# lanl/jaybenne

Measured on AMD Instinct MI355X. Metric: particle-histories/s (whole node) on stepdiff, higher is better.
Workload: dtype f64

## Files before the change

jaybenne_amd/csrc/jb_kernel_imc.hpp:

```cpp
#pragma once

#include "jb_kernels.hpp"

namespace jb {

#ifndef JB_IMC_WAVES_PER_SIMD_UNIFORM
#define JB_IMC_WAVES_PER_SIMD_UNIFORM 4
#endif
#ifndef JB_IMC_WAVES_PER_SIMD
#define JB_IMC_WAVES_PER_SIMD 4
#endif
#ifndef JB_IMC_WAVES_PER_SIMD_LOWD
#define JB_IMC_WAVES_PER_SIMD_LOWD 4
#endif
#ifndef JB_IMC_NT_STORES
#define JB_IMC_NT_STORES 0
#endif
#ifndef JB_IMC_MASKED_NUDGE
#define JB_IMC_MASKED_NUDGE 1
#endif
#ifndef JB_IMC_SERVICE_BUDGET
#define JB_IMC_SERVICE_BUDGET 96
#endif

struct ImcArgs {
  const DevMesh *Mp;
  DevParams P;
  DevSwarm S;
  double t_start, dt;
  long long first, last;
  unsigned long long *counters;
  const int *nbr_dq;
};

enum { IS_IDLE = 0, IS_RUN = 1, IS_DONE = 2, IS_DONE_RAW = 3 };
#ifndef JB_IMC_WIDE_LOG
#define JB_IMC_WIDE_LOG 1
#endif
constexpr bool kWideLog = JB_IMC_WIDE_LOG != 0;


template <int NDIM, bool TALLY, bool NOABS, bool UNIFORM>
__global__ void __launch_bounds__(kBlock, NDIM < 3 ? JB_IMC_WAVES_PER_SIMD_LOWD
                                          : UNIFORM ? JB_IMC_WAVES_PER_SIMD_UNIFORM : JB_IMC_WAVES_PER_SIMD)
    k_imc_cell(const DevMesh *__restrict__, DevParams, DevSwarm, double, double, long long, long long,
               unsigned long long *, const int *) {
  const ImcArgs &A = *(const ImcArgs *)__builtin_amdgcn_kernarg_segment_ptr();
  const DevMesh &M = *A.Mp;
  const DevParams &P = A.P;
  const DevSwarm &S = A.S;
  const double t_start = A.t_start, dt = A.dt;
  const long long first = A.first, last = A.last;
  unsigned long long *const counters = g1(A.counters);
  (void)A.nbr_dq;
  constexpr bool multi_d = NDIM >= 2, three_d = NDIM == 3;
  __shared__ double lds_tally[TALLY ? kLdsTally : 1];
  const bool tally_in_lds = TALLY && (long long)M.nblocks * M.ntot <= (long long)kLdsTally;
  if constexpr (TALLY) {
    if (tally_in_lds)
      for (int q = threadIdx.x; q < M.nblocks * (int)M.ntot; q += blockDim.x) lds_tally[q] = 0.0;
  }
  constexpr bool kWide = kWideLog && NOABS;
  constexpr bool kMasked = JB_IMC_MASKED_NUDGE != 0;
  load_math_tables<false, !kWide, false, true, kWide>();

  constexpr int kServiceBudget = JB_IMC_SERVICE_BUDGET;
  const double vv = P.c;
  const double t_end = t_start + dt;
  const int lane = threadIdx.x & 63;
  unsigned long long *queue = counters + CNT_QUEUE;
  const long long per_q = (last - first + kQueues - 1) / kQueues;
  int cur = blockIdx.x % kQueues;
  int tried = 0;
  bool more = true;

  unsigned int c_census = 0, c_abs = 0, c_esc = 0, c_out = 0;
  unsigned long long c_evp = 0;
  unsigned int c_service = 0;

  const int sy = (int)sgpr_copy(8u * (unsigned)M.ni), sz = (int)sgpr_copy(8u * (unsigned)(M.ni * M.nj));
  const unsigned blk_bytes = 16u * (unsigned)M.ntot;
  const char *const lam_abs0 = (const char *)sgpr_copy_ptr(M.lam_base);
  const char *const lam_sc0 = (const char *)sgpr_copy_ptr(M.lam_base + M.ntot);
  const double inv_ni = 1.0 / (double)M.ni, inv_ninj = 1.0 / (double)(M.ni * M.nj);
  const double inv_blk_bytes = 1.0 / (double)blk_bytes;

  int ls = IS_IDLE;
  long long n = 0;
  LcgRng rng(0);
  int b = 0, status = ST_ACTIVE;
  unsigned qoff = 0u;
  double px = 0, py = 0, pz = 0;
  double ox = 0, oy = 0, oz = 0;
  double drem = 0;
  CellGeom cg{0, 0, 0, 0, 0, 0, 0};
  if constexpr (UNIFORM) {
    const double d0 = uniform_f64(M.blk_dx[0]), d1 = uniform_f64(M.blk_dx[1]), d2 = uniform_f64(M.blk_dx[2]);
    cg.hx = 0.5 * d0; cg.hy = 0.5 * d1; cg.hz = 0.5 * d2;
    cg.mx = cg.hx - kEpsImc * d0; cg.my = cg.hy - kEpsImc * d1; cg.mz = cg.hz - kEpsImc * d2;
    cg.dxp = dmin(d0, dmin(d1, d2));
  }
  double lam_a = 0.0, lam_s = 0.0;
  JB_INV_STMT(bool inv_collided = false;)

  auto fetch_lam = [&]() {
    if constexpr (!NOABS) lam_a = *(gcptr)(lam_abs0 + qoff);
    lam_s = *(gcptr)(lam_sc0 + qoff);
  };
  auto bind_block = [&](int blk) {
    if constexpr (UNIFORM) return;
    const double d0 = ((gcptr)M.blk_dx)[3 * blk], d1 = ((gcptr)M.blk_dx)[3 * blk + 1],
                 d2 = ((gcptr)M.blk_dx)[3 * blk + 2];
    cg.hx = 0.5 * d0; cg.hy = 0.5 * d1; cg.hz = 0.5 * d2;
    cg.mx = cg.hx - kEpsImc * d0; cg.my = cg.hy - kEpsImc * d1; cg.mz = cg.hz - kEpsImc * d2;
    cg.dxp = dmin(d0, dmin(d1, d2));
  };
  auto block_of = [&]() { return (int)(((double)qoff + 4.0) * inv_blk_bytes); };
  auto cell_of = [&](int &i, int &j, int &k) {
    const int q = (int)((qoff - (unsigned)b * blk_bytes) >> 3);
    k = three_d ? (int)(((double)q + 0.5) * inv_ninj) : 0;
    const int r = q - k * (M.ni * M.nj);
    j = multi_d ? (int)(((double)r + 0.5) * inv_ni) : 0;
    i = r - j * M.ni;
  };
  auto centre = [&](int blk, int d, int idx) {
    const double dxd = ((gcptr)M.blk_dx)[3 * blk + d];
    const int first_d = d == 0 ? M.is : (d == 1 ? M.js : M.ks);
    const double x0 = ((gcptr)M.blk_xmin)[3 * blk + d] - (double)first_d * dxd;
    return fma((double)idx + 0.5, dxd, x0);
  };
  auto materialise = [&](double &x, double &y, double &z, int &i, int &j, int &k) {
    cell_of(i, j, k);
    x = centre(b, 0, i) + px;
    y = multi_d ? centre(b, 1, j) + py : py;
    z = three_d ? centre(b, 2, k) + pz : pz;
  };
  auto localise = [&](double x, double y, double z, int i, int j, int k) {
    px = x - centre(b, 0, i);
    py = multi_d ? y - centre(b, 1, j) : y;
    pz = three_d ? z - centre(b, 2, k) : z;
    qoff = (unsigned)b * blk_bytes + ((unsigned)cidx(M, k, j, i) << 3);
  };
  bool abs_pos = false;
  auto relocate = [&]() {
    double x, y, z;
    int i, j, k;
    materialise(x, y, z, i, j, k);
    if (!apply_swarm_bcs<NDIM>(M, x, y, z, ox, oy, oz)) {
      status = ST_ESCAPED;
      px = x; py = y; pz = z;
      abs_pos = true;
      ls = IS_DONE;
      return;
    }
    const int g = find_block<NDIM>(M, x, y, z);
    const int li = M.local_index[g];
    if (li < 0) {
      status = ST_OUTGOING;
      b = g;
      px = x; py = y; pz = z;
      abs_pos = true;
      ls = IS_DONE;
      return;
    }
    b = li;
    bind_block(b);
    Blk B;
    load_block(M, b, B);
    xtoijk<NDIM>(M, B, x, y, z, i, j, k);
    localise(x, y, z, i, j, k);
    ls = (drem > 0.0) ? IS_RUN : IS_DONE;
    fetch_lam();
  };

  for (;;) {
    ++c_service;
    if (ls == IS_DONE || ls == IS_DONE_RAW) {
      double x = px, y = py, z = pz;
      int ip = 0, jp = 0, kp = 0;
      if (!abs_pos) {
        b = block_of();
        materialise(x, y, z, ip, jp, kp);
      }
      double t = drem, vx = ox, vy = oy, vz = oz;
      if (ls == IS_DONE) {
        t = fma(-drem, P.rc, t_end);
        vx *= vv; vy *= vv; vz *= vv;
      }
      int bw = b;
      if (!abs_pos && (status == ST_ACTIVE || status == ST_OUTGOING_ABSORBED) && !M.owned[b]) {
        if (status == ST_ACTIVE) status = ST_OUTGOING;
        bw = M.gid[b];
      }
#if JB_IMC_NT_STORES
#define JB_WST(p, v) __builtin_nontemporal_store((v), (p))
#else
#define JB_WST(p, v) (*(p) = (v))
#endif
      JB_WST(&g1(S.blk)[n], bw);
      JB_WST(&g1(S.t)[n], t);
      JB_WST(&g1(S.x)[n], x); JB_WST(&g1(S.y)[n], y); JB_WST(&g1(S.z)[n], z);
      JB_WST(&g1(S.vx)[n], vx); JB_WST(&g1(S.vy)[n], vy); JB_WST(&g1(S.vz)[n], vz);
      JB_WST(&g1(S.ip)[n], ip); JB_WST(&g1(S.jp)[n], jp); JB_WST(&g1(S.kp)[n], kp);
      JB_WST(&g1(S.status)[n], status);
      JB_WST(&g1(S.rng)[n], (uint64_t)rng.s);
#undef JB_WST
      if (status == ST_ACTIVE) {
        ++c_census;
        if constexpr (TALLY) {
          const double dv = (8.0 * cg.hx) * cg.hy * cg.hz;
          const int q = (int)((qoff - (unsigned)b * blk_bytes) >> 3);
          if (tally_in_lds) atomicAdd(&lds_tally[b * (int)M.ntot + q], g1(S.w)[n] / dv);
          else atomicAdd(&M.tally[b][q], g1(S.w)[n] / dv);
        }
      } else if (status == ST_ABSORBED) {
        ++c_abs;
      } else if (status == ST_ESCAPED) {
        ++c_esc;
      } else {
        ++c_out;
      }
      ls = IS_IDLE;
      abs_pos = false;
    }
    {
      const unsigned long long idle = __ballot(ls == IS_IDLE);
      if (idle != 0ull && more) {
        const int leader = __ffsll((long long)idle) - 1;
        const int want = __popcll(idle);
        unsigned long long base = 0;
        if (lane == leader) base = atomicAdd(&queue[cur * kQueueStride], (unsigned long long)want);
        base = __shfl(base, leader, 64);
        const long long q_first = first + (long long)cur * per_q;
        long long q_last = q_first + per_q;
        if (q_last > last) q_last = last;
        const long long cand = q_first + (long long)base + __popcll(idle & ((1ull << lane) - 1ull));
        if (q_first + (long long)base + want >= q_last) {
          cur = (cur + 1) % kQueues;
          if (++tried == kQueues) more = false;
        }
        if (ls == IS_IDLE && cand < q_last && g1(S.status)[cand] == ST_ACTIVE) {
          n = cand;
          rng.s = g1(S.rng)[n];
          b = g1(S.blk)[n];
          bind_block(b);
          const double t = g1(S.t)[n];
          const double x = g1(S.x)[n], y = g1(S.y)[n], z = g1(S.z)[n];
          ox = g1(S.vx)[n]; oy = g1(S.vy)[n]; oz = g1(S.vz)[n];
          status = ST_ACTIVE;
          Blk B;
          load_block(M, b, B);
          int i, j, k;
          xtoijk<NDIM>(M, B, x, y, z, i, j, k);
          localise(x, y, z, i, j, k);
          if (t < t_end) {
            drem = vv * (t_end - t);
            ox *= P.rc; oy *= P.rc; oz *= P.rc;
            ls = IS_RUN;
          } else {
            drem = t;
            ls = IS_DONE_RAW;
          }
          fetch_lam();
        }
      }
    }
    const int running = __popcll(__ballot(ls == IS_RUN));
    if (running == 0) {
      if (__ballot(ls != IS_IDLE) != 0ull || more) continue;
      break;
    }
    int waste = 0;

    int thresh = 1;
    int nrun = running;
    while (nrun >= thresh) {
      const bool run = ls == IS_RUN;
      const bool cross = run && lam_s < 0.0;
      const bool stepping = run && !cross;
      const unsigned long long cross_m =
          __builtin_amdgcn_ballot_w64(ls == IS_RUN) & __builtin_amdgcn_ballot_w64(lam_s < 0.0);
      c_evp += (1ull << 40) + (unsigned long long)(nrun - __popcll(cross_m));
      if (cross_m != 0ull) {
        if (cross) {
          JB_INV_OFF_BLOCK(JB_INV_FAM_IMC_CELL, inv_collided, false, block_of(), 0, 0, 0, px, py, pz, n, S.id, (void)0);
          const int code = __double2hiint(lam_s);
          if ((code & kGhostTable) == 0) {
            b = block_of();
            relocate();
          } else {
            const int fx = (code << 15) & (int)0x80000000u, fy = (code << 14) & (int)0x80000000u,
                      fz = (code << 13) & (int)0x80000000u;
            px = __hiloint2double(__double2hiint(px) ^ fx, __double2loint(px));
            ox = __hiloint2double(__double2hiint(ox) ^ fx, __double2loint(ox));
            if (multi_d) {
              py = __hiloint2double(__double2hiint(py) ^ fy, __double2loint(py));
              oy = __hiloint2double(__double2hiint(oy) ^ fy, __double2loint(oy));
            }
            if (three_d) {
              pz = __hiloint2double(__double2hiint(pz) ^ fz, __double2loint(pz));
              oz = __hiloint2double(__double2hiint(oz) ^ fz, __double2loint(oz));
            }
            qoff = (unsigned)__double2loint(lam_s);
            if constexpr (!UNIFORM) {
              if (code & (kGhostCoarser | kGhostFiner))
                qoff = cross_level<NDIM>(code, qoff, sy, sz, cg, px, py, pz);
            }
            fetch_lam();
            if (!(drem > 0.0)) ls = IS_DONE;
          }
        }
      }
      JB_INV_STMT(bool inv_bad = false;)
      JB_INV_STMT({
        int ib = -1, ii = 0, ij = 0, ik = 0, ax = 0;
        const double pp[3] = {px, py, pz}, hh[3] = {cg.hx, cg.hy, cg.hz};
        const bool pos = inv::local_position_ok(NDIM, pp, hh, ax);
        const unsigned cell = (qoff % blk_bytes) >> 3;
        const bool idx = cell < (unsigned)M.ntot &&
                         inv::cell_interior(M, (unsigned long long)(qoff / blk_bytes) * (unsigned long long)M.ntot + cell,
                                            ib, ii, ij, ik);
        JB_INV_PASS_PRED(JB_INV_FAM_IMC_CELL, stepping, pos, idx, ax, ib, ii, ij, ik, px, py, pz, n, S.id,
                         { inv_bad = true; ls = IS_IDLE; });
      })
      if (stepping JB_INV_STMT(&& !inv_bad)) {
        bool is_absorbed, is_scattered, hit_any;
        unsigned long long hit_m;
        imc_step_cell<NDIM, NOABS, UNIFORM, kWide, kMasked>(cg, sy, sz, lam_a, lam_s, rng, drem, px, py, pz, ox, oy, oz,
                                                     qoff, is_absorbed, is_scattered, hit_any, &hit_m, fetch_lam);
        const bool alive = drem > 0.0, census = !alive;
        bool collide = is_absorbed || is_scattered;
        bool off = false;
        const unsigned long long at_face_m =
            hit_m & (__builtin_amdgcn_ballot_w64(collide) | ~__builtin_amdgcn_ballot_w64(alive));
        const bool at_face = __builtin_amdgcn_inverse_ballot_w64(at_face_m);
        if (at_face_m != 0ull) {
          asm volatile("; collision or census next to a cell face" ::: "memory");
          if (at_face) off = lam_s < 0.0;
        }
        collide = collide && !off;
        JB_INV_STMT(inv_collided = collide;)
        if (!NOABS && is_absorbed && collide) {
          b = block_of();
          if (M.owned[b]) {
            atomicAdd(&M.edelta[b][(qoff - (unsigned)b * blk_bytes) >> 3], g1(S.w)[n]);
            status = ST_ABSORBED;
          } else {
            status = ST_OUTGOING_ABSORBED;
          }
          ls = IS_DONE;
        } else {
          if (is_scattered && collide) scatter_dir<true>(rng, ox, oy, oz);
          if (census && !off) ls = IS_DONE;
        }
      }
      nrun = __popcll(__ballot(ls == IS_RUN));
      waste += running - nrun;
      if (waste >= kServiceBudget) thresh = 65;
    }
  }

  if constexpr (TALLY) {
    if (tally_in_lds) {
      __syncthreads();
      for (int q = threadIdx.x; q < M.nblocks * (int)M.ntot; q += blockDim.x) {
        const double v = lds_tally[q];
        if (v != 0.0) atomicAdd(&M.tally[q / (int)M.ntot][q % (int)M.ntot], v);
      }
    }
  }
  unsigned long long r_census = wave_sum(c_census), r_abs = wave_sum(c_abs), r_esc = wave_sum(c_esc),
                     r_out = wave_sum(c_out);
  if (lane == 0) {
    if (r_census) atomicAdd(&counters[CNT_CENSUS], r_census);
    if (r_abs) atomicAdd(&counters[CNT_ABSORBED], r_abs);
    if (r_esc) atomicAdd(&counters[CNT_ESCAPED], r_esc);
    if (r_out) atomicAdd(&counters[CNT_OUTGOING], r_out);
    atomicAdd(&counters[CNT_EVENTS], c_evp & ((1ull << 40) - 1ull));
    atomicAdd(&counters[CNT_PASSES], c_evp >> 40);
    atomicAdd(&counters[CNT_SERVICE], (unsigned long long)c_service);
  }
}

}
```

jaybenne_amd/csrc/jb_physics.hpp:

```cpp
#pragma once

#include <float.h>
#include <hip/hip_runtime.h>

#include "jb_math.hpp"
#include "jb_rng.hpp"

namespace jb {

constexpr double kEps = 10.0 * DBL_EPSILON;
constexpr double kEpsImc = 1.0e6 * kEps;
constexpr double kEpsDdmc = 1.0e8 * kEps;
constexpr double kLamExt = 0.7104;
constexpr double kTwoPi = 2.0 * 3.14159265358979323846;

__device__ __forceinline__ double dmin(double a, double b) { return (b < a) ? b : a; }

__device__ __forceinline__ bool fuzzy_equal(double a, double b, double c, double eps) {
  return fabs(a - b) < c * eps;
}

__device__ __forceinline__ void face_iso_dir(double vv, double xi1, double xi2, double &v1,
                                             double &v2, double &v3) {
  const double mu = m_sqrt(xi1);
  const double om = 1.0 - mu * mu;
  const double nu = (om > 0.0) ? m_sqrt(om > 0.0 ? om : 1.0) : 0.0;
  double sn, cs;
  m_sincos2pi(xi2, sn, cs);
  v1 = vv * mu;
  v2 = vv * nu * cs;
  v3 = vv * nu * sn;
}

template <class Rng>
__device__ __forceinline__ void sample_face_iso_dir(double vv, Rng &rng, double &v1, double &v2,
                                                    double &v3) {
  const double xi1 = rng.drand();
  const double xi2 = rng.drand();
  face_iso_dir(vv, xi1, xi2, v1, v2, v3);
}

template <class Rng>
__device__ __forceinline__ void scatter(Rng &rng, double vv, double &vx, double &vy, double &vz) {
  double xi1, xi2;
  rng.drand2(xi1, xi2);
  const double mu = fma(2.0, xi1, -1.0);
  const double st = m_sqrt(1.0 - mu * mu);
  double sn, cs;
  m_sincos2pi(xi2, sn, cs);
  vx = vv * st * cs;
  vy = vv * st * sn;
  vz = vv * mu;
}

template <class Rng>
__device__ __forceinline__ double sample_planck_energy(Rng &rng, double sb, double temp) {
  constexpr double kPi = 3.14159265358979323846;
  const double xi0 = rng.drand();
  const double rhs = xi0 * ((kPi * kPi) * (kPi * kPi)) / 90.0;
  double ll = 1.0;
  for (int l = 1; l < 100; ++l) {
    double lhs = 0.0;
    for (int j = 1; j <= l; ++j) {
      const double dj = (double)j;
      lhs += 1.0 / ((dj * dj) * (dj * dj));
    }
    if (lhs >= rhs) {
      ll = (double)l;
      break;
    }
  }
  const double xi1 = rng.drand();
  const double xi2 = rng.drand();
  const double xi3 = rng.drand();
  const double xi4 = rng.drand();
  return -(1.0 / ll) * m_log(xi1 * xi2 * xi3 * xi4) * sb * temp;
}

struct Step {
  double t_start, dt;
  double ff, aa, ss, vv, dx_push;
  double rvv;
  double ffaa, sig;
  double xl, yl, zl, xu, yu, zu;
  double Px_l, Py_l, Pz_l, Px_u, Py_u, Pz_u;
  double t, x, y, z, vx, vy, vz;
  int ip, jp, kp;
  bool is_absorbed, is_scattered, is_rejected;
  int pend;
  double pz1, pz2;
};

__device__ __forceinline__ void imc_cell_mfp(double ff, double aa, double ss, double &lam_abs,
                                             double &lam_sc) {
  const double rmin = DBL_MIN;
  lam_abs = 1.0 / (ff * aa + rmin);
  lam_sc = 1.0 / (ss + (1.0 - ff) * aa + rmin);
}

template <int NDIM, bool NOABS = false, class Rng>
__device__ __forceinline__ void imc_step_core(Step &s, double lam_abs, double lam_sc, Rng &rng) {
  constexpr bool multi_d = NDIM >= 2, three_d = NDIM == 3;
  double dx_abs = 0.0;
  if constexpr (NOABS) rng.skip();
  else dx_abs = -lam_abs * m_log(rng.drand());
  const double dx_sc = -lam_sc * m_log(rng.drand());
  const double dx_end = s.vv * ((s.t_start + s.dt) - s.t);
  double dx_push = dmin(s.dx_push, dx_end);
  {
    const double d = m_div(s.vv * ((s.vx > 0.0 ? s.xu : s.xl) - s.x), s.vx);
    dx_push = (s.vx != 0.0) ? dmin(dx_push, d) : dx_push;
  }
  if (multi_d) {
    const double d = m_div(s.vv * ((s.vy > 0.0 ? s.yu : s.yl) - s.y), s.vy);
    dx_push = (s.vy != 0.0) ? dmin(dx_push, d) : dx_push;
  }
  if (three_d) {
    const double d = m_div(s.vv * ((s.vz > 0.0 ? s.zu : s.zl) - s.z), s.vz);
    dx_push = (s.vz != 0.0) ? dmin(dx_push, d) : dx_push;
  }

  s.is_absorbed = NOABS ? false : (dx_abs < dx_push) && (dx_abs < dx_sc);
  s.is_scattered = !s.is_absorbed && (dx_sc < dx_push);

  const double dt_push = m_div_r(s.is_absorbed ? dx_abs : (s.is_scattered ? dx_sc : dx_push), s.vv,
                                 s.rvv);

  s.t += dt_push;
  s.x += s.vx * dt_push;
  s.y += (multi_d ? 1.0 : 0.0) * s.vy * dt_push;
  s.z += (three_d ? 1.0 : 0.0) * s.vz * dt_push;

  const double fdx = kEpsImc * (s.xu - s.xl);
  const double fdy = kEpsImc * (s.yu - s.yl);
  const double fdz = kEpsImc * (s.zu - s.zl);
  if (fabs(s.x - s.xl) < fdx) s.x = s.xl - fdx;
  if (fabs(s.x - s.xu) < fdx) s.x = s.xu + fdx;
  if (multi_d && fabs(s.y - s.yl) < fdy) s.y = s.yl - fdy;
  if (multi_d && fabs(s.y - s.yu) < fdy) s.y = s.yu + fdy;
  if (three_d && fabs(s.z - s.zl) < fdz) s.z = s.zl - fdz;
  if (three_d && fabs(s.z - s.zu) < fdz) s.z = s.zu + fdz;
}

__device__ __forceinline__ void idx_step(int &i, bool hi, bool lo) {
  i += (int)hi;
  i -= (int)lo;
}

struct ImcCell {
  double xl, xu, yl, yu, zl, zu;
  double fdx, fdy, fdz;
};
template <int NDIM, bool NOABS, bool LEAN = false, class Rng>
__device__ __forceinline__ void imc_step_fast(const ImcCell &c, double vv, double rvv, double t_end,
                                              double dx_push0, double lam_abs, double lam_sc,
                                              Rng &rng, double &t, double &x, double &y, double &z,
                                              double vx, double vy, double vz, int &ip, int &jp,
                                              int &kp, bool &is_absorbed, bool &is_scattered) {
  constexpr bool multi_d = NDIM >= 2, three_d = NDIM == 3;
  double dx_abs = 0.0;
  if constexpr (NOABS) rng.skip();
  else dx_abs = -lam_abs * (LEAN ? m_log_lean(rng.drand()) : m_log(rng.drand()));
  const double dx_sc = -lam_sc * (LEAN ? m_log_lean(rng.drand()) : m_log(rng.drand()));
  const double dx_end = vv * (t_end - t);
  double dx_push = m_min(dx_push0, dx_end);
  if constexpr (LEAN) {
    dx_push = m_min(dx_push, (vv * ((vx > 0.0 ? c.xu : c.xl) - x)) * m_rcp_once(vx));
    if (multi_d) dx_push = m_min(dx_push, (vv * ((vy > 0.0 ? c.yu : c.yl) - y)) * m_rcp_once(vy));
    if (three_d) dx_push = m_min(dx_push, (vv * ((vz > 0.0 ? c.zu : c.zl) - z)) * m_rcp_once(vz));
  } else {
    dx_push = m_min(dx_push, m_div(vv * ((vx > 0.0 ? c.xu : c.xl) - x), vx));
    if (multi_d) dx_push = m_min(dx_push, m_div(vv * ((vy > 0.0 ? c.yu : c.yl) - y), vy));
    if (three_d) dx_push = m_min(dx_push, m_div(vv * ((vz > 0.0 ? c.zu : c.zl) - z), vz));
  }
  is_absorbed = NOABS ? false : (dx_abs < dx_push) && (dx_abs < dx_sc);
  is_scattered = !is_absorbed && (dx_sc < dx_push);
  const double dx_move =
      NOABS ? m_min(dx_push, dx_sc) : (is_absorbed ? dx_abs : (is_scattered ? dx_sc : dx_push));
  if constexpr (LEAN) {
    const double dt_push = dx_move * rvv;
    t += dt_push;
    x = fma(vx, dt_push, x);
    if (multi_d) y = fma(vy, dt_push, y);
    if (three_d) z = fma(vz, dt_push, z);
  } else {
    const double dt_push = m_div_r(dx_move, vv, rvv);
    t += dt_push;
    x += vx * dt_push;
    y += (multi_d ? 1.0 : 0.0) * vy * dt_push;
    z += (three_d ? 1.0 : 0.0) * vz * dt_push;
  }
  {
    const bool lo = fabs(x - c.xl) < c.fdx, hi = fabs(x - c.xu) < c.fdx;
    x = lo ? c.xl - c.fdx : (hi ? c.xu + c.fdx : x);
    idx_step(ip, hi, lo);
  }
  if (multi_d) {
    const bool lo = fabs(y - c.yl) < c.fdy, hi = fabs(y - c.yu) < c.fdy;
    y = lo ? c.yl - c.fdy : (hi ? c.yu + c.fdy : y);
    idx_step(jp, hi, lo);
  }
  if (three_d) {
    const bool lo = fabs(z - c.zl) < c.fdz, hi = fabs(z - c.zu) < c.fdz;
    z = lo ? c.zl - c.fdz : (hi ? c.zu + c.fdz : z);
    idx_step(kp, hi, lo);
  }
}

struct DirGeom {
  double x0[3], dx[3], fd[3];
};
__device__ __forceinline__ bool dir_up(double o) { return __double2hiint(o) >= 0; }
template <bool EXACTG>
__device__ __forceinline__ double dir_face(const DirGeom &g, int d, int idx, bool up, int &iu) {
  iu = idx + (int)up;
  if constexpr (EXACTG) {
    return m_fma((double)iu, g.dx[d], g.x0[d]);
  } else {
    const double xcd = g.x0[d] + ((double)idx + 0.5) * g.dx[d];
    return up ? xcd + 0.5 * g.dx[d] : xcd - 0.5 * g.dx[d];
  }
}
__device__ __forceinline__ void dir_nudge(double &x, int &idx, double o, double f, double fd, int iu,
                                          bool up) {
  const bool hit = fabs(x - f) < fd;
  int shi;
  asm("v_bfi_b32 %0, %1, %2, %3" : "=v"(shi) : "s"(0x7fffffff), "v"(__double2hiint(fd)), "v"(__double2hiint(o)));
  x = hit ? f + __hiloint2double(shi, __double2loint(fd)) : x;
  idx = iu - (int)(hit != up);
}
__device__ __forceinline__ void dir_nudge_carried(double &x, int &idx, double o, double f, double &sfd,
                                                  int iu, bool up) {
  int shi;
  asm("v_bfi_b32 %0, %1, %2, %3" : "=v"(shi) : "s"(0x7fffffff), "v"(__double2hiint(sfd)), "v"(__double2hiint(o)));
  sfd = __hiloint2double(shi, __double2loint(sfd));
  const bool hit = fabs(x - f) < fabs(sfd);
  x = hit ? f + sfd : x;
  idx = iu - (int)(hit != up);
}
__device__ __forceinline__ void dir_nudge_behind(double &x, int &idx, double fb, double fd, bool up) {
  const bool hit = fabs(x - fb) < fd;
  x = hit ? (up ? fb - fd : fb + fd) : x;
  idx += hit ? (up ? -1 : 1) : 0;
}
template <int NDIM, bool NOABS, bool EXACTG, bool BOTH = false, class Rng>
__device__ __forceinline__ void imc_step_dir(DirGeom &g, double dx_push0, double lam_abs,
                                             double lam_sc, Rng &rng, double &d_rem, double &x,
                                             double &y, double &z, double ox, double oy, double oz,
                                             int &ip, int &jp, int &kp, bool &is_absorbed,
                                             bool &is_scattered) {
  constexpr bool multi_d = NDIM >= 2, three_d = NDIM == 3;
  double dx_abs = 0.0;
  if constexpr (NOABS) rng.skip();
  else dx_abs = -lam_abs * m_log_lean(rng.drand());
  const double dx_sc = -lam_sc * m_log_lean(rng.drand());
  double dx_push = m_min(dx_push0, d_rem);
  const bool upx = dir_up(ox), upy = dir_up(oy), upz = dir_up(oz);
  int iux = 0, iuy = 0, iuz = 0;
  const double fx = dir_face<EXACTG>(g, 0, ip, upx, iux);
  const double fy = multi_d ? dir_face<EXACTG>(g, 1, jp, upy, iuy) : 0.0;
  const double fz = three_d ? dir_face<EXACTG>(g, 2, kp, upz, iuz) : 0.0;
#ifndef JB_NO_PRODUCT_RCP
  if constexpr (three_d) {
    const double pxy = ox * oy, q = pxy * oz;
    double rx, ry, rz;
    if (fabs(q) > 1.0e-250) {
      const double r = m_rcp_once(q);
      const double roz = r * oz;
      rz = r * pxy; rx = roz * oy; ry = roz * ox;
    } else {
      rx = m_rcp_once(ox); ry = m_rcp_once(oy); rz = m_rcp_once(oz);
    }
    dx_push = m_min(dx_push, (fx - x) * rx);
    dx_push = m_min(dx_push, (fy - y) * ry);
    dx_push = m_min(dx_push, (fz - z) * rz);
  } else
#endif
  {
    dx_push = m_min(dx_push, (fx - x) * m_rcp_once(ox));
    if (multi_d) dx_push = m_min(dx_push, (fy - y) * m_rcp_once(oy));
    if (three_d) dx_push = m_min(dx_push, (fz - z) * m_rcp_once(oz));
  }
  is_absorbed = NOABS ? false : (dx_abs < dx_push) && (dx_abs < dx_sc);
  is_scattered = !is_absorbed && (dx_sc < dx_push);
  const double dx_move =
      NOABS ? m_min(dx_push, dx_sc) : (is_absorbed ? dx_abs : (is_scattered ? dx_sc : dx_push));
  d_rem -= dx_move;
  x = fma(ox, dx_move, x);
  if (multi_d) y = fma(oy, dx_move, y);
  if (three_d) z = fma(oz, dx_move, z);
  if constexpr (EXACTG) {
    dir_nudge_carried(x, ip, ox, fx, g.fd[0], iux, upx);
    if (multi_d) dir_nudge_carried(y, jp, oy, fy, g.fd[1], iuy, upy);
    if (three_d) dir_nudge_carried(z, kp, oz, fz, g.fd[2], iuz, upz);
  } else {
    dir_nudge(x, ip, ox, fx, kEpsImc * g.dx[0], iux, upx);
    if (multi_d) dir_nudge(y, jp, oy, fy, kEpsImc * g.dx[1], iuy, upy);
    if (three_d) dir_nudge(z, kp, oz, fz, kEpsImc * g.dx[2], iuz, upz);
  }
  if constexpr (BOTH) {
    int unused;
    dir_nudge_behind(x, ip, dir_face<EXACTG>(g, 0, iux - (int)upx, !upx, unused), kEpsImc * g.dx[0], upx);
    if (multi_d)
      dir_nudge_behind(y, jp, dir_face<EXACTG>(g, 1, iuy - (int)upy, !upy, unused), kEpsImc * g.dx[1], upy);
    if (three_d)
      dir_nudge_behind(z, kp, dir_face<EXACTG>(g, 2, iuz - (int)upz, !upz, unused), kEpsImc * g.dx[2], upz);
  }
}

template <bool M_UNIFORM = false>
__device__ __forceinline__ double nudged(double p, double m, bool hit) {
#ifdef JB_NO_ASM_NUDGE
  return hit ? -copysign(m, p) : p;
#else
#ifdef JB_UNIFORM_NUDGE_CXX
  if constexpr (M_UNIFORM) return hit ? -copysign(m, p) : p;
#endif
  const unsigned long long mask = __ballot(hit);
  int chi, hi, lo;
  asm("v_bfi_b32 %0, %1, %2, %3" : "=v"(chi) : "s"(0x7fffffff), "v"(__double2hiint(m)), "v"(__double2hiint(p)));
  asm("v_cndmask_b32_e64 %0, %1, -%2, %3" : "=v"(hi) : "v"(__double2hiint(p)), "v"(chi), "s"(mask));
  asm("v_cndmask_b32_e64 %0, %1, %2, %3" : "=v"(lo) : "v"(__double2loint(p)), "v"(__double2loint(m)), "s"(mask));
  return __hiloint2double(hi, lo);
#endif
}

#ifdef JB_NO_ASM_NUDGE
constexpr bool kMaskedNudge = false;
#else
constexpr bool kMaskedNudge = true;
#endif
typedef unsigned long long lane_mask;
#define JB_NUDGE_AXIS(a)                                                                      \
  "v_med3_i32 %[t], %[h" a "], -1, 1\n\tv_mad_i32_i24 %[q], %[t], %[s" a "], %[q]\n\t"        \
  "v_bfi_b32 %[h" a "], %[k], %[mh" a "], %[h" a "]\n\tv_xor_b32_e32 %[h" a "], 0x80000000, %[h" a "]\n\t" \
  "v_mov_b32_e32 %[l" a "], %[ml" a "]\n\t"
template <int NDIM>
__device__ __forceinline__ void nudge_reindex_masked(double &px, double &py, double &pz, unsigned &qoff, double mx,
                                                     double my, double mz, int sy, int sz, lane_mask hx,
                                                     lane_mask hy, lane_mask hz) {
  lane_mask sv;
  int t;
  int hix = __double2hiint(px), lox = __double2loint(px);
  if constexpr (NDIM == 1) {
    asm("s_and_saveexec_b64 %[sv], %[mx]\n\t" JB_NUDGE_AXIS("x") "s_mov_b64 exec, %[sv]"
        : [sv] "=&s"(sv), [t] "=&v"(t), [q] "+v"(qoff), [hx] "+v"(hix), [lx] "+v"(lox)
        : [mx] "s"(hx), [k] "s"(0x7fffffff), [sx] "n"(8), [mhx] "v"(__double2hiint(mx)),
          [mlx] "v"(__double2loint(mx))
        : "scc");
  } else if constexpr (NDIM == 2) {
    int hiy = __double2hiint(py), loy = __double2loint(py);
    asm("s_and_saveexec_b64 %[sv], %[mx]\n\t" JB_NUDGE_AXIS("x")
        "s_and_b64 exec, %[sv], %[my]\n\t" JB_NUDGE_AXIS("y") "s_mov_b64 exec, %[sv]"
        : [sv] "=&s"(sv), [t] "=&v"(t), [q] "+v"(qoff), [hx] "+v"(hix), [lx] "+v"(lox), [hy] "+v"(hiy),
          [ly] "+v"(loy)
        : [mx] "s"(hx), [my] "s"(hy), [k] "s"(0x7fffffff), [sx] "n"(8), [sy] "s"(sy),
          [mhx] "v"(__double2hiint(mx)), [mlx] "v"(__double2loint(mx)), [mhy] "v"(__double2hiint(my)),
          [mly] "v"(__double2loint(my))
        : "scc");
    py = __hiloint2double(hiy, loy);
  } else {
    int hiy = __double2hiint(py), loy = __double2loint(py), hiz = __double2hiint(pz), loz = __double2loint(pz);
    asm("s_and_saveexec_b64 %[sv], %[mx]\n\t" JB_NUDGE_AXIS("x")
        "s_and_b64 exec, %[sv], %[my]\n\t" JB_NUDGE_AXIS("y")
        "s_and_b64 exec, %[sv], %[mz]\n\t" JB_NUDGE_AXIS("z") "s_mov_b64 exec, %[sv]"
        : [sv] "=&s"(sv), [t] "=&v"(t), [q] "+v"(qoff), [hx] "+v"(hix), [lx] "+v"(lox), [hy] "+v"(hiy),
          [ly] "+v"(loy), [hz] "+v"(hiz), [lz] "+v"(loz)
        : [mx] "s"(hx), [my] "s"(hy), [mz] "s"(hz), [k] "s"(0x7fffffff), [sx] "n"(8), [sy] "s"(sy), [sz] "s"(sz),
          [mhx] "v"(__double2hiint(mx)), [mlx] "v"(__double2loint(mx)), [mhy] "v"(__double2hiint(my)),
          [mly] "v"(__double2loint(my)), [mhz] "v"(__double2hiint(mz)), [mlz] "v"(__double2loint(mz))
        : "scc");
    py = __hiloint2double(hiy, loy);
    pz = __hiloint2double(hiz, loz);
  }
  px = __hiloint2double(hix, lox);
}
#undef JB_NUDGE_AXIS
struct NoGather {
  __device__ __forceinline__ void operator()() const {}
};

struct CellGeom {
  double hx, hy, hz, mx, my, mz, dxp;
};
template <int NDIM, bool NOABS, bool UNIFORM = false, bool WIDELOG = false, bool MASKED = false, class Rng,
          class Gather = NoGather>
__device__ __forceinline__ void imc_step_cell(const CellGeom &g, int sy, int sz, double lam_a, double lam_s,
                                              Rng &rng, double &drem, double &px, double &py, double &pz,
                                              double ox, double oy, double oz, unsigned &qoff,
                                              bool &is_absorbed, bool &is_scattered, bool &hit_any,
                                              unsigned long long *hit_mask = nullptr, Gather gather = Gather()) {
  constexpr bool multi_d = NDIM >= 2, three_d = NDIM == 3;
  constexpr int sx = 8;
  double dx_abs = 0.0;
  if constexpr (NOABS) rng.skip();
  else dx_abs = -lam_a * m_log_lean<true, WIDELOG>(rng.drand());
  const double dx_sc = -lam_s * m_log_lean<true, WIDELOG>(rng.drand());
#ifdef JB_IMC_NO_SCALAR_MIN
  double dx_push = m_min(g.dxp, drem);
#else
  double dx_push = UNIFORM ? m_min_s(g.dxp, drem) : m_min(g.dxp, drem);
#endif
  double rx, ry = 0.0, rz = 0.0;
  if constexpr (three_d) {
    const double pxy = ox * oy, q = pxy * oz;
    if (fabs(q) > 1.0e-250) {
      const double r = m_rcp_once(q);
      const double roz = r * oz;
      rz = r * pxy; rx = roz * oy; ry = roz * ox;
    } else {
      rx = m_rcp_once(ox); ry = m_rcp_once(oy); rz = m_rcp_once(oz);
    }
  } else {
    rx = m_rcp_once(ox);
    if (multi_d) ry = m_rcp_once(oy);
  }
  dx_push = m_min(dx_push, m_fnma(px, rx, g.hx * fabs(rx)));
  if (multi_d) dx_push = m_min(dx_push, m_fnma(py, ry, g.hy * fabs(ry)));
  if (three_d) dx_push = m_min(dx_push, m_fnma(pz, rz, g.hz * fabs(rz)));
  is_absorbed = NOABS ? false : (dx_abs < dx_push) && (dx_abs < dx_sc);
  is_scattered = !is_absorbed && (dx_sc < dx_push);
  const double dx_move =
      NOABS ? m_min(dx_push, dx_sc) : (is_absorbed ? dx_abs : (is_scattered ? dx_sc : dx_push));
  drem -= dx_move;
  px = fma(ox, dx_move, px);
  if (multi_d) py = fma(oy, dx_move, py);
  if (three_d) pz = fma(oz, dx_move, pz);
  if constexpr (MASKED && kMaskedNudge) {
    const lane_mask hx = __builtin_amdgcn_ballot_w64(fabs(px) > g.mx);
    const lane_mask hy = multi_d ? __builtin_amdgcn_ballot_w64(fabs(py) > g.my) : 0ull;
    const lane_mask hz = three_d ? __builtin_amdgcn_ballot_w64(fabs(pz) > g.mz) : 0ull;
    const lane_mask hm = hx | hy | hz;
    hit_any = __builtin_amdgcn_inverse_ballot_w64(hm);
    if (hit_mask) *hit_mask = hm;
    nudge_reindex_masked<NDIM>(px, py, pz, qoff, g.mx, g.my, g.mz, sy, sz, hx, hy, hz);
    if (hit_any) gather();
    return;
  }
  const bool hit_x = fabs(px) > g.mx;
  const bool hit_y = multi_d && fabs(py) > g.my;
  const bool hit_z = three_d && fabs(pz) > g.mz;
  auto side = [](double p) { return (__double2hiint(p) >> 31) | 1; };
  qoff = (unsigned)mad24(hit_x ? side(px) : 0, sx, (int)qoff);
  px = nudged<UNIFORM>(px, g.mx, hit_x);
  if (multi_d) {
    qoff = (unsigned)mad24(hit_y ? side(py) : 0, sy, (int)qoff);
    py = nudged<UNIFORM>(py, g.my, hit_y);
  }
  if (three_d) {
    qoff = (unsigned)mad24(hit_z ? side(pz) : 0, sz, (int)qoff);
    pz = nudged<UNIFORM>(pz, g.mz, hit_z);
  }
  hit_any = hit_x || hit_y || hit_z;
  if (hit_mask) {
    unsigned long long m = __builtin_amdgcn_ballot_w64(hit_x);
    if (multi_d) m |= __builtin_amdgcn_ballot_w64(hit_y);
    if (three_d) m |= __builtin_amdgcn_ballot_w64(hit_z);
    *hit_mask = m;
  }
  if (hit_any) gather();
}

template <int NDIM>
__device__ __forceinline__ unsigned cross_level(int code, unsigned dst, int sy, int sz, CellGeom &g, double &px,
                                                double &py, double &pz) {
  constexpr bool multi_d = NDIM >= 2, three_d = NDIM == 3;
  if (code & 0x100) {
    px += (code & 0x400) ? -g.hx : g.hx;
    if (multi_d) py += (code & 0x800) ? -g.hy : g.hy;
    if (three_d) pz += (code & 0x1000) ? -g.hz : g.hz;
    g.hx *= 2.0; g.mx *= 2.0;
    if (multi_d) { g.hy *= 2.0; g.my *= 2.0; }
    if (three_d) { g.hz *= 2.0; g.mz *= 2.0; }
    g.dxp = dmin(2.0 * g.hx, dmin(2.0 * g.hy, 2.0 * g.hz));
    return dst;
  }
  g.hx *= 0.5; g.mx *= 0.5;
  if (multi_d) { g.hy *= 0.5; g.my *= 0.5; }
  if (three_d) { g.hz *= 0.5; g.mz *= 0.5; }
  g.dxp = dmin(2.0 * g.hx, dmin(2.0 * g.hy, 2.0 * g.hz));
  const int naxis = (code >> 10) & 3;
  const bool lower = (code & 0x1000) != 0;
  {
    const bool up = !(px < 0.0);
    if (naxis == 0) px += lower ? -g.hx : g.hx;
    else { px += up ? -g.hx : g.hx; dst += up ? 8u : 0u; }
  }
  if (multi_d) {
    const bool up = !(py < 0.0);
    if (naxis == 1) py += lower ? -g.hy : g.hy;
    else { py += up ? -g.hy : g.hy; dst += up ? (unsigned)sy : 0u; }
  }
  if (three_d) {
    const bool up = !(pz < 0.0);
    if (naxis == 2) pz += lower ? -g.hz : g.hz;
    else { pz += up ? -g.hz : g.hz; dst += up ? (unsigned)sz : 0u; }
  }
  return dst;
}

template <bool SC = false, class Rng>
__device__ __forceinline__ void scatter_dir(Rng &rng, double &ox, double &oy, double &oz) {
  double xi1, xi2;
  rng.drand2(xi1, xi2);
  const double mu = fma(2.0, xi1, -1.0);
  const double st = m_sqrt_lean(1.0 - mu * mu);
  double sn, cs;
  m_sincos2pi<SC>(xi2, sn, cs);
  ox = st * cs;
  oy = st * sn;
  oz = mu;
}

template <int NDIM, class Rng>
__device__ __forceinline__ void ptcl_transport_step(Step &s, Rng &rng) {
  double lam_abs, lam_sc;
  imc_cell_mfp(s.ff, s.aa, s.ss, lam_abs, lam_sc);
  imc_step_core<NDIM, false>(s, lam_abs, lam_sc, rng);
}

__device__ __forceinline__ void assign_cyclic(int axis, double v1, double v2, double v3, double &vx,
                                              double &vy, double &vz) {
  vx = (axis == 0) ? v1 : (axis == 1 ? v3 : v2);
  vy = (axis == 0) ? v2 : (axis == 1 ? v1 : v3);
  vz = (axis == 0) ? v3 : (axis == 1 ? v2 : v1);
}

__device__ __forceinline__ void materialise_dir(Step &s) {
  const int axis = s.pend >> 1;
  const bool up = (s.pend & 1) != 0;
  double v1, v2, v3;
  face_iso_dir(up ? s.vv : -s.vv, s.pz1, s.pz2, v1, v2, v3);
  assign_cyclic(axis, v1, v2, v3, s.vx, s.vy, s.vz);
  s.pend = -1;
}

template <int NDIM, bool LEAK_READY = false, bool LAZY = false, bool PRELOG = false, class Rng>
__device__ __forceinline__ bool ddmc_step_event(Step &s, Rng &rng, double nlog = 0.0) {
  constexpr int multi_d = NDIM >= 2 ? 1 : 0, three_d = NDIM == 3 ? 1 : 0;
  const double rmin = DBL_MIN;
  const double eps = kEpsDdmc;
  const double dx = s.xu - s.xl;
  const double dy = s.yu - s.yl;
  const double dz = s.zu - s.zl;

  const double leakx_l = LEAK_READY ? s.Px_l : s.Px_l / dx;
  const double leakx_u = LEAK_READY ? s.Px_u : s.Px_u / dx;
  const double leaky_l = LEAK_READY ? s.Py_l : s.Py_l / dy;
  const double leaky_u = LEAK_READY ? s.Py_u : s.Py_u / dy;
  const double leakz_l = LEAK_READY ? s.Pz_l : s.Pz_l / dz;
  const double leakz_u = LEAK_READY ? s.Pz_u : s.Pz_u / dz;
  const double leak_tot = leakx_l + leakx_u + leaky_l + leaky_u + leakz_l + leakz_u;

  const double cdf_ddmc = s.ffaa + leak_tot + rmin;
  if constexpr (!PRELOG) nlog = -m_log(rng.drand());
  const double dt_ddmc = m_div(nlog, s.vv * cdf_ddmc);
  const double dt_end = (s.t_start + s.dt) - s.t;
  const bool is_ddmc_event = dt_ddmc < dt_end;

  s.t += dmin(dt_ddmc, dt_end);

  if (is_ddmc_event) {
    const double xi = cdf_ddmc * rng.drand();
    if (xi < s.ffaa) {
      s.is_absorbed = true;
    } else if (xi < s.ffaa + leak_tot) {
      const double xim = xi - s.ffaa;
      const double c1 = leakx_l;
      const double c2 = leakx_l + leakx_u;
      const double c3 = c2 + leaky_l;
      const double c4 = c3 + leaky_u;
      const double c5 = c4 + leakz_l;
      const int ch = (xim < c1) ? 0 : (xim < c2) ? 1 : (xim < c3) ? 2 : (xim < c4) ? 3
                   : (xim < c5) ? 4 : (xim <= leak_tot) ? 5 : -1;
      if (ch >= 0) {
        const int axis = ch >> 1;
        const bool up = (ch & 1) != 0;
        const int step = up ? 1 : -1;
        s.ip += (axis == 0) ? step : 0;
        s.jp += (axis == 1) ? step * multi_d : 0;
        s.kp += (axis == 2) ? step * three_d : 0;
        s.x = (axis == 0) ? (up ? s.xu + eps * dx : s.xl - eps * dx) : s.xl + 0.5 * dx;
        s.y = (axis == 1) ? (up ? s.yu + eps * dy : s.yl - eps * dy) : s.yl + 0.5 * dy;
        s.z = (axis == 2) ? (up ? s.zu + eps * dz : s.zl - eps * dz) : s.zl + 0.5 * dz;
        if constexpr (LAZY) {
          s.pz1 = rng.drand();
          s.pz2 = rng.drand();
          s.pend = ch;
        } else {
          double v1, v2, v3;
          sample_face_iso_dir(up ? s.vv : -s.vv, rng, v1, v2, v3);
          assign_cyclic(axis, v1, v2, v3, s.vx, s.vy, s.vz);
        }
      }
    }
  }
  return !is_ddmc_event;
}

struct DdmcStepRec {
  double ffaa, c1, c2, c3, c4, c5, leak_tot, rcp;
};
template <int NDIM, class Rng>
__device__ __forceinline__ bool ddmc_step_rec(const DdmcStepRec &r, double vv, double dt_end, double nlog,
                                              Rng &rng, double &t, int &ip, int &jp, int &kp, int &pend,
                                              unsigned long long &pzs, bool &is_absorbed) {
  constexpr int multi_d = NDIM >= 2 ? 1 : 0, three_d = NDIM == 3 ? 1 : 0;
  const double a2 = r.ffaa + r.leak_tot;
  const double cdf_ddmc = a2 + DBL_MIN;
  const double dt_ddmc = m_div_r(nlog, vv * cdf_ddmc, r.rcp);
  const bool is_ddmc_event = dt_ddmc < dt_end;
  t += dmin(dt_ddmc, dt_end);
  if (is_ddmc_event) {
    const double xi = cdf_ddmc * rng.drand();
    if (xi < r.ffaa) {
      is_absorbed = true;
    } else if (xi < a2) {
      const double xim = xi - r.ffaa;
      int ch = (xim <= r.leak_tot) ? 5 : -1;
      if constexpr (three_d) ch = (xim < r.c5) ? 4 : ch;
      if constexpr (multi_d) {
        ch = (xim < r.c4) ? 3 : ch;
        ch = (xim < r.c3) ? 2 : ch;
      }
      ch = (xim < r.c2) ? 1 : ch;
      ch = (xim < r.c1) ? 0 : ch;
      if (ch >= 0) {
        const int axis = ch >> 1;
        const int step = (ch & 1) != 0 ? 1 : -1;
        ip += (axis == 0) ? step : 0;
        jp += (axis == 1) ? step * multi_d : 0;
        kp += (axis == 2) ? step * three_d : 0;
        pzs = rng.s;
        rng.skip2();
        pend = ch;
      }
    }
  }
  return !is_ddmc_event;
}

template <class Rng>
__device__ __forceinline__ void ddmc_census_resample(Step &s, Rng &rng) {
  const double dx = s.xu - s.xl;
  const double dy = s.yu - s.yl;
  const double dz = s.zu - s.zl;
  s.z = s.zl + rng.drand() * dz;
  s.x = s.xl + rng.drand() * dx;
  s.y = s.yl + rng.drand() * dy;
  const double mu = 1.0 - 2.0 * rng.drand();
  const double nu = sqrt(1.0 - mu * mu);
  const double xi2 = rng.drand();
  double sn, cs;
  m_sincos2pi(xi2, sn, cs);
  s.vz = s.vv * mu;
  s.vx = s.vv * nu * cs;
  s.vy = s.vv * nu * sn;
}

template <int NDIM, class Rng>
__device__ __forceinline__ void ptcl_ddmc_step(Step &s, Rng &rng) {
  if (ddmc_step_event<NDIM, false, false>(s, rng)) ddmc_census_resample(s, rng);
}

template <int NDIM, bool LAZY = false, class Rng>
__device__ __forceinline__ void ptcl_ddmc_albedo(Step &s, Rng &rng) {
  constexpr bool multi_d = NDIM >= 2, three_d = NDIM == 3;
  const double dx = s.xu - s.xl;
  const double dy = s.yu - s.yl;
  const double dz = s.zu - s.zl;
  const double tol = 2.5 * kEpsImc;

  int face = -1;
  if (fuzzy_equal(s.x, s.xl, dx, tol)) face = 0;
  else if (fuzzy_equal(s.x, s.xu, dx, tol)) face = 1;
  else if (multi_d && fuzzy_equal(s.y, s.yl, dy, tol)) face = 2;
  else if (multi_d && fuzzy_equal(s.y, s.yu, dy, tol)) face = 3;
  else if (three_d && fuzzy_equal(s.z, s.zl, dz, tol)) face = 4;
  else if (three_d && fuzzy_equal(s.z, s.zu, dz, tol)) face = 5;

  if (face >= 0) {
    if constexpr (LAZY) {
      if (s.pend >= 0) materialise_dir(s);
    }
    const int axis = face >> 1;
    const double sgn = (face & 1) ? -1.0 : 1.0;
    const double svx = s.vx, svy = s.vy, svz = s.vz;
    const double sxl = s.xl, sxu = s.xu, syl = s.yl, syu = s.yu, szl = s.zl, szu = s.zu;
    const bool upper = (face & 1) != 0;
    const double dcell = (axis == 0) ? dx : (axis == 1 ? dy : dz);
    const double vn = (axis == 0) ? svx : (axis == 1 ? svy : svz);
    const double fx = upper ? sxu : sxl, fy = upper ? syu : syl, fz = upper ? szu : szl;
    const double fpos = (axis == 0) ? fx : (axis == 1 ? fy : fz);
    const double Pf = (2.0 / 3.0) / (s.sig * dcell + 2.0 * kLamExt);
    const double P = 2.0 * Pf * (1.0 + sgn * 1.5 * vn / s.vv);
    if (rng.drand() > P) {
      double v1, v2, v3;
      sample_face_iso_dir(-sgn * s.vv, rng, v1, v2, v3);
      assign_cyclic(axis, v1, v2, v3, s.vx, s.vy, s.vz);
      const double xn = fpos - sgn * kEpsImc * dcell;
      if (axis == 0) s.x = xn;
      else if (axis == 1) s.y = xn;
      else s.z = xn;
      s.is_rejected = true;
    }
  }

  if (!s.is_rejected) {
    s.x = 0.5 * (s.xl + s.xu);
    s.y = 0.5 * (s.yl + s.yu);
    s.z = 0.5 * (s.zl + s.zu);
  }
}

template <int NDIM>
__device__ __forceinline__ bool at_cell_face(const Step &s) {
  constexpr bool multi_d = NDIM >= 2, three_d = NDIM == 3;
  const double dx = s.xu - s.xl, dy = s.yu - s.yl, dz = s.zu - s.zl;
  const double tol = 2.5 * kEpsImc;
  return fuzzy_equal(s.x, s.xl, dx, tol) || fuzzy_equal(s.x, s.xu, dx, tol) ||
         (multi_d && (fuzzy_equal(s.y, s.yl, dy, tol) || fuzzy_equal(s.y, s.yu, dy, tol))) ||
         (three_d && (fuzzy_equal(s.z, s.zl, dz, tol) || fuzzy_equal(s.z, s.zu, dz, tol)));
}

template <class Rng>
__device__ __forceinline__ void sample_face_2d(int i_l, double dx, double P_l, double P_u, Rng &rng,
                                               int &i, double &x) {
  const double xi = (P_l + P_u) * rng.drand();
  if (xi < P_l) {
    x -= dx * rng.drand();
    i = i_l;
  } else {
    x += dx * rng.drand();
    i = i_l + 1;
  }
}

template <class Rng>
__device__ __forceinline__ void sample_face_3d(int i1_l, int i2_l, double dx1, double dx2,
                                               double P_ll, double P_lu, double P_ul, double P_uu,
                                               Rng &rng, int &i1, int &i2, double &x1, double &x2) {
  const double xi = (P_ll + P_lu + P_ul + P_uu) * rng.drand();
  if (xi < P_ll) {
    x1 -= dx1 * rng.drand(); i1 = i1_l;
    x2 -= dx2 * rng.drand(); i2 = i2_l;
  } else if (xi < P_ll + P_lu) {
    x1 += dx1 * rng.drand(); i1 = i1_l + 1;
    x2 -= dx2 * rng.drand(); i2 = i2_l;
  } else if (xi < P_ll + P_lu + P_ul) {
    x1 -= dx1 * rng.drand(); i1 = i1_l;
    x2 += dx2 * rng.drand(); i2 = i2_l + 1;
  } else {
    x1 += dx1 * rng.drand(); i1 = i1_l + 1;
    x2 += dx2 * rng.drand(); i2 = i2_l + 1;
  }
}

}
```

Baseline: 198.5 million.

## Track IMC run state as wave-wide scalar lane masks in the inner step loop

Replaces the per-lane run/cross/stepping booleans in the inner transport loop with wave-uniform lane masks (run_m, step_m, scat_m, abs_m, census_m) held in scalar registers, so the loop count and branch decisions come from scalar ballot arithmetic rather than repeated per-lane comparisons and ballots. The step kernel is split so the movement part can be called separately and the collision classification is recomputed from masks. Wall mirroring is factored into a lambda that skips the sign-flip work when no lane in the wave hits a reflecting wall. This adds complexity and uses asm-volatile tricks to leave registers undefined on inactive lanes, which risks subtle correctness issues. The old vector-state path remains available behind a macro.

New measurement: 200.4 million, median of 6. No clear change (+1.0%).

```diff
diff --git a/jaybenne_amd/csrc/jb_kernel_imc.hpp b/jaybenne_amd/csrc/jb_kernel_imc.hpp
--- a/jaybenne_amd/csrc/jb_kernel_imc.hpp
+++ b/jaybenne_amd/csrc/jb_kernel_imc.hpp
@@ -21,6 +21,13 @@
 #endif
 #ifndef JB_IMC_SERVICE_BUDGET
 #define JB_IMC_SERVICE_BUDGET 96
+#endif
+#ifndef JB_IMC_WALL_BRANCH
+#ifdef JB_IMC_VECTOR_STATE
+#define JB_IMC_WALL_BRANCH 0
+#else
+#define JB_IMC_WALL_BRANCH 1
+#endif
 #endif
 
 struct ImcArgs {
@@ -62,6 +69,7 @@
   }
   constexpr bool kWide = kWideLog && NOABS;
   constexpr bool kMasked = JB_IMC_MASKED_NUDGE != 0;
+  constexpr bool kWallBranch = JB_IMC_WALL_BRANCH != 0;
   load_math_tables<false, !kWide, false, true, kWide>();
 
   constexpr int kServiceBudget = JB_IMC_SERVICE_BUDGET;
@@ -171,6 +179,22 @@
     localise(x, y, z, i, j, k);
     ls = (drem > 0.0) ? IS_RUN : IS_DONE;
     fetch_lam();
+  };
+
+  auto wall_mirror = [&](int code) {
+    if (kWallBranch && __builtin_amdgcn_ballot_w64((code & 0x70000) != 0) == 0ull) return;
+    const int fx = (code << 15) & (int)0x80000000u, fy = (code << 14) & (int)0x80000000u,
+              fz = (code << 13) & (int)0x80000000u;
+    px = __hiloint2double(__double2hiint(px) ^ fx, __double2loint(px));
+    ox = __hiloint2double(__double2hiint(ox) ^ fx, __double2loint(ox));
+    if (multi_d) {
+      py = __hiloint2double(__double2hiint(py) ^ fy, __double2loint(py));
+      oy = __hiloint2double(__double2hiint(oy) ^ fy, __double2loint(oy));
+    }
+    if (three_d) {
+      pz = __hiloint2double(__double2hiint(pz) ^ fz, __double2loint(pz));
+      oz = __hiloint2double(__double2hiint(oz) ^ fz, __double2loint(oz));
+    }
   };
 
   for (;;) {
@@ -274,6 +298,107 @@
 
     int thresh = 1;
     int nrun = running;
+#ifndef JB_IMC_VECTOR_STATE
+    lane_mask run_m = __builtin_amdgcn_ballot_w64(ls == IS_RUN);
+    while (nrun >= thresh) {
+      const lane_mask ghost_m = __builtin_amdgcn_ballot_w64(lam_s < 0.0);
+      const lane_mask cross_m = run_m & ghost_m;
+      lane_mask step_m = run_m & ~ghost_m;
+      c_evp += (1ull << 40) + (unsigned long long)__popcll(step_m);
+      if (cross_m != 0ull) {
+        if (__builtin_amdgcn_inverse_ballot_w64(cross_m)) {
+          JB_INV_OFF_BLOCK(JB_INV_FAM_IMC_CELL, inv_collided, false, block_of(), 0, 0, 0, px, py, pz, n, S.id, (void)0);
+          const int code = __double2hiint(lam_s);
+          if ((code & kGhostTable) == 0) {
+            b = block_of();
+            relocate();
+          } else {
+            wall_mirror(code);
+            qoff = (unsigned)__double2loint(lam_s);
+            if constexpr (!UNIFORM) {
+              if (code & (kGhostCoarser | kGhostFiner))
+                qoff = cross_level<NDIM>(code, qoff, sy, sz, cg, px, py, pz);
+            }
+            fetch_lam();
+            if (!(drem > 0.0)) ls = IS_DONE;
+          }
+        }
+        run_m &= __builtin_amdgcn_ballot_w64(ls == IS_RUN);
+      }
+      JB_INV_STMT(bool inv_bad = false;)
+      JB_INV_STMT({
+        const bool stepping = __builtin_amdgcn_inverse_ballot_w64(step_m);
+        int ib = -1, ii = 0, ij = 0, ik = 0, ax = 0;
+        const double pp[3] = {px, py, pz}, hh[3] = {cg.hx, cg.hy, cg.hz};
+        const bool pos = inv::local_position_ok(NDIM, pp, hh, ax);
+        const unsigned cell = (qoff % blk_bytes) >> 3;
+        const bool idx = cell < (unsigned)M.ntot &&
+                         inv::cell_interior(M, (unsigned long long)(qoff / blk_bytes) * (unsigned long long)M.ntot + cell,
+                                            ib, ii, ij, ik);
+        JB_INV_PASS_PRED(JB_INV_FAM_IMC_CELL, stepping, pos, idx, ax, ib, ii, ij, ik, px, py, pz, n, S.id,
+                         { inv_bad = true; ls = IS_IDLE; });
+        const lane_mask bad_m = __builtin_amdgcn_ballot_w64(inv_bad);
+        step_m &= ~bad_m;
+        run_m &= ~bad_m;
+      })
+      lane_mask scat_m, abs_m = 0ull, hit_m;
+      if constexpr (kMasked && kMaskedNudge) {
+        double dx_abs = 0.0, dx_sc, dx_push;
+        if constexpr (!NOABS) asm volatile("; dx_abs: the register as it stands" : "=v"(dx_abs));
+        asm volatile("; dx_sc, dx_push: the registers as they stand" : "=v"(dx_sc), "=v"(dx_push));
+        if (__builtin_amdgcn_inverse_ballot_w64(step_m)) {
+          bool is_absorbed, is_scattered;
+          imc_step_move<NDIM, NOABS, UNIFORM, kWide>(cg, lam_a, lam_s, rng, drem, px, py, pz, ox, oy, oz, is_absorbed,
+                                                     is_scattered, dx_abs, dx_sc, dx_push);
+        }
+        if constexpr (!NOABS)
+          abs_m = step_m & __builtin_amdgcn_ballot_w64(dx_abs < dx_push) & __builtin_amdgcn_ballot_w64(dx_abs < dx_sc);
+        scat_m = step_m & ~abs_m & __builtin_amdgcn_ballot_w64(dx_sc < dx_push);
+        const lane_mask hx = step_m & __builtin_amdgcn_ballot_w64(fabs(px) > cg.mx);
+        const lane_mask hy = multi_d ? step_m & __builtin_amdgcn_ballot_w64(fabs(py) > cg.my) : 0ull;
+        const lane_mask hz = three_d ? step_m & __builtin_amdgcn_ballot_w64(fabs(pz) > cg.mz) : 0ull;
+        hit_m = hx | hy | hz;
+        nudge_reindex_masked<NDIM>(px, py, pz, qoff, cg.mx, cg.my, cg.mz, sy, sz, hx, hy, hz);
+        if (__builtin_amdgcn_inverse_ballot_w64(hit_m)) fetch_lam();
+      } else {
+        bool is_absorbed = false, is_scattered = false, hit_any = false;
+        if (__builtin_amdgcn_inverse_ballot_w64(step_m)) {
+          imc_step_cell<NDIM, NOABS, UNIFORM, kWide, kMasked>(cg, sy, sz, lam_a, lam_s, rng, drem, px, py, pz, ox, oy,
+                                                              oz, qoff, is_absorbed, is_scattered, hit_any, nullptr,
+                                                              fetch_lam);
+        }
+        scat_m = step_m & __builtin_amdgcn_ballot_w64(is_scattered);
+        if constexpr (!NOABS) abs_m = step_m & __builtin_amdgcn_ballot_w64(is_absorbed);
+        hit_m = step_m & __builtin_amdgcn_ballot_w64(hit_any);
+      }
+      const lane_mask census_m = step_m & ~__builtin_amdgcn_ballot_w64(drem > 0.0);
+      const lane_mask at_face_m = hit_m & (scat_m | abs_m | census_m);
+      lane_mask off_m = 0ull;
+      if (at_face_m != 0ull) {
+        asm volatile("; collision or census next to a cell face" ::: "memory");
+        off_m = at_face_m & __builtin_amdgcn_ballot_w64(lam_s < 0.0);
+      }
+      JB_INV_STMT(if (__builtin_amdgcn_inverse_ballot_w64(step_m))
+                      inv_collided = __builtin_amdgcn_inverse_ballot_w64((scat_m | abs_m) & ~off_m);)
+      if constexpr (!NOABS) {
+        if (__builtin_amdgcn_inverse_ballot_w64(abs_m & ~off_m)) {
+          b = block_of();
+          if (M.owned[b]) {
+            atomicAdd(&M.edelta[b][(qoff - (unsigned)b * blk_bytes) >> 3], g1(S.w)[n]);
+            status = ST_ABSORBED;
+          } else {
+            status = ST_OUTGOING_ABSORBED;
+          }
+        }
+      }
+      if (__builtin_amdgcn_inverse_ballot_w64(scat_m & ~off_m)) scatter_dir<true>(rng, ox, oy, oz);
+      run_m &= ~((abs_m | census_m) & ~off_m);
+      nrun = __popcll(run_m);
+      waste += running - nrun;
+      if (waste >= kServiceBudget) thresh = 65;
+    }
+    if (ls == IS_RUN && !__builtin_amdgcn_inverse_ballot_w64(run_m)) ls = IS_DONE;
+#else
     while (nrun >= thresh) {
       const bool run = ls == IS_RUN;
       const bool cross = run && lam_s < 0.0;
@@ -289,18 +414,7 @@
             b = block_of();
             relocate();
           } else {
-            const int fx = (code << 15) & (int)0x80000000u, fy = (code << 14) & (int)0x80000000u,
-                      fz = (code << 13) & (int)0x80000000u;
-            px = __hiloint2double(__double2hiint(px) ^ fx, __double2loint(px));
-            ox = __hiloint2double(__double2hiint(ox) ^ fx, __double2loint(ox));
-            if (multi_d) {
-              py = __hiloint2double(__double2hiint(py) ^ fy, __double2loint(py));
-              oy = __hiloint2double(__double2hiint(oy) ^ fy, __double2loint(oy));
-            }
-            if (three_d) {
-              pz = __hiloint2double(__double2hiint(pz) ^ fz, __double2loint(pz));
-              oz = __hiloint2double(__double2hiint(oz) ^ fz, __double2loint(oz));
-            }
+            wall_mirror(code);
             qoff = (unsigned)__double2loint(lam_s);
             if constexpr (!UNIFORM) {
               if (code & (kGhostCoarser | kGhostFiner))
@@ -358,6 +472,7 @@
       waste += running - nrun;
       if (waste >= kServiceBudget) thresh = 65;
     }
+#endif
   }
 
   if constexpr (TALLY) {
diff --git a/jaybenne_amd/csrc/jb_physics.hpp b/jaybenne_amd/csrc/jb_physics.hpp
--- a/jaybenne_amd/csrc/jb_physics.hpp
+++ b/jaybenne_amd/csrc/jb_physics.hpp
@@ -383,23 +383,20 @@
 struct CellGeom {
   double hx, hy, hz, mx, my, mz, dxp;
 };
-template <int NDIM, bool NOABS, bool UNIFORM = false, bool WIDELOG = false, bool MASKED = false, class Rng,
-          class Gather = NoGather>
-__device__ __forceinline__ void imc_step_cell(const CellGeom &g, int sy, int sz, double lam_a, double lam_s,
-                                              Rng &rng, double &drem, double &px, double &py, double &pz,
-                                              double ox, double oy, double oz, unsigned &qoff,
-                                              bool &is_absorbed, bool &is_scattered, bool &hit_any,
-                                              unsigned long long *hit_mask = nullptr, Gather gather = Gather()) {
+template <int NDIM, bool NOABS, bool UNIFORM = false, bool WIDELOG = false, class Rng>
+__device__ __forceinline__ void imc_step_move(const CellGeom &g, double lam_a, double lam_s, Rng &rng, double &drem,
+                                              double &px, double &py, double &pz, double ox, double oy, double oz,
+                                              bool &is_absorbed, bool &is_scattered, double &dx_abs, double &dx_sc,
+                                              double &dx_push) {
   constexpr bool multi_d = NDIM >= 2, three_d = NDIM == 3;
-  constexpr int sx = 8;
-  double dx_abs = 0.0;
+  dx_abs = 0.0;
   if constexpr (NOABS) rng.skip();
   else dx_abs = -lam_a * m_log_lean<true, WIDELOG>(rng.drand());
-  const double dx_sc = -lam_s * m_log_lean<true, WIDELOG>(rng.drand());
+  dx_sc = -lam_s * m_log_lean<true, WIDELOG>(rng.drand());
 #ifdef JB_IMC_NO_SCALAR_MIN
-  double dx_push = m_min(g.dxp, drem);
+  dx_push = m_min(g.dxp, drem);
 #else
-  double dx_push = UNIFORM ? m_min_s(g.dxp, drem) : m_min(g.dxp, drem);
+  dx_push = UNIFORM ? m_min_s(g.dxp, drem) : m_min(g.dxp, drem);
 #endif
   double rx, ry = 0.0, rz = 0.0;
   if constexpr (three_d) {
@@ -426,6 +423,20 @@
   px = fma(ox, dx_move, px);
   if (multi_d) py = fma(oy, dx_move, py);
   if (three_d) pz = fma(oz, dx_move, pz);
+}
+
+template <int NDIM, bool NOABS, bool UNIFORM = false, bool WIDELOG = false, bool MASKED = false, class Rng,
+          class Gather = NoGather>
+__device__ __forceinline__ void imc_step_cell(const CellGeom &g, int sy, int sz, double lam_a, double lam_s,
+                                              Rng &rng, double &drem, double &px, double &py, double &pz,
+                                              double ox, double oy, double oz, unsigned &qoff,
+                                              bool &is_absorbed, bool &is_scattered, bool &hit_any,
+                                              unsigned long long *hit_mask = nullptr, Gather gather = Gather()) {
+  constexpr bool multi_d = NDIM >= 2, three_d = NDIM == 3;
+  constexpr int sx = 8;
+  double dx_abs, dx_sc, dx_push;
+  imc_step_move<NDIM, NOABS, UNIFORM, WIDELOG>(g, lam_a, lam_s, rng, drem, px, py, pz, ox, oy, oz, is_absorbed,
+                                               is_scattered, dx_abs, dx_sc, dx_push);
   if constexpr (MASKED && kMaskedNudge) {
     const lane_mask hx = __builtin_amdgcn_ballot_w64(fabs(px) > g.mx);
     const lane_mask hy = multi_d ? __builtin_amdgcn_ballot_w64(fabs(py) > g.my) : 0ull;
```
